# blachlylab/fade

Measured on AMD Instinct MI355X. Metric: annotate reads/sec at 1/2/4/8 MI355X; rs/am tag bit-exact vs ref, higher is better.
Workload: dtype int16; 1 GPU; C2: 10000000 x 150 bp PE reads per GPU per step in 10 distinct batches, -w 100, --min-length 5, p_softclip 0.10; slots_in_flight=2, records_left_out=none

## Files before the change

fade_amd/csrc/fadehip.hip:

```cpp
#include "fadehip_host.hpp"
#include "fadehip_kernels.hpp"
#include "sw_stats.hpp"
#include <fcntl.h>
#include <sys/stat.h>
#include <unistd.h>
#include <algorithm>
#include <cerrno>
#include <climits>
#include <cstdio>
#include <cstdlib>
#include <cstring>
#include <string>
#include <thread>
#include <vector>

using namespace fadehip;
using namespace fadehip::host;

namespace {

int reserve_run(fadehip_ctx *ctx, std::vector<void *> &trash, DevBuf &b, size_t bytes) {
    if (bytes <= b.cap && b.p) return 0;
    if (b.p) trash.push_back(b.p);
    b.p = nullptr;
// ... 219 lines not shown
    int64_t chunk_oct = 1;
    int total_oct = 0;
    uint64_t wave_stride = 0;
    int p2_waves = 1;
    size_t ckpt_bytes = 0, fwd_bytes = 0, trace_bytes = 0, cand_bytes = 0;
};

int plan_two_pass(fadehip_ctx *ctx, const Slot &s, const ClassRun &c, TwoPassPlan &p) {
    const int cls = c.cls, R = class_rows(cls), max_lr = c.max_lr, n_items = c.n_bound;
    p.n_ck = s.use_ckpt ? (max_lr + 15 + CK_COLS - 1) / CK_COLS : 0;
    p.ck_stride = (uint64_t)p.n_ck * ck_dwords(R) * 64;
    p.n_blocks1 = (max_lr + 15 + 3) / 4;
    p.ref_stride1 = std::min((((p.n_blocks1 * 4) * 2 + 15) / 16) * 16, (CH_COLS + 16) * 2);
    p.lds1 = (size_t)p.ref_stride1 * 4;
    const bool alt_rules = (ctx->sc.rules & (FADEHIP_RULE_HDIR_DIAG_F_E | FADEHIP_RULE_GAP_TIE_EXTENDS)) !=
                           (FADEHIP_RULE_HDIR_DIAG_F_E | FADEHIP_RULE_GAP_TIE_EXTENDS);
    p.mode2 = alt_rules ? 3 : 2;
    const int64_t ck_bytes = (int64_t)p.ck_stride * 4;
    p.total_oct = (n_items + 7) / 8;
    p.chunk_oct = std::max<int64_t>(1, std::min<int64_t>(p.total_oct, (c.budget / 2) / std::max<int64_t>(ck_bytes, 1)));
    p.wave_stride = (uint64_t)p.n_blocks1 * R * 64;
    p.longw = p.n_blocks1 > CH_BLOCKS;
    const int resident = resident_waves(ctx, cls, p.mode2, p.lds1, p.longw);
    const int bound_waves = (int)std::min<int64_t>(p.chunk_oct + NUM_BUCKETS, resident);
    int p2_waves = s.p2_last_octs[cls] >= 0 ? std::min(2 * s.p2_last_octs[cls] + 64, bound_waves) : std::min(1024, bound_waves);
    if (ctx->p2_waves_fixed > 0) p2_waves = std::min(ctx->p2_waves_fixed, bound_waves);
    p.p2_waves = (int)std::max<int64_t>(1, std::min<int64_t>(p2_waves, (c.budget / 2) / std::max<int64_t>((int64_t)p.wave_stride * 4, 1)));
    p.ckpt_bytes = (size_t)(p.chunk_oct * ck_bytes);
    p.fwd_bytes = (size_t)n_items * sizeof(Fwd);
    p.trace_bytes = (size_t)p.p2_waves * (size_t)p.wave_stride * 4;
    p.cand_bytes = sizeof(Cand) * (size_t)NUM_BUCKETS * (size_t)std::min<int64_t>(n_items, p.chunk_oct * 8);
    return 0;
}

int run_class_two_pass(fadehip_ctx *ctx, Slot &s, hipStream_t st, const ClassRun &c) {
    const int cls = c.cls, n_items = c.n_bound;
    TwoPassPlan p;
    int rc;
    if ((rc = plan_two_pass(ctx, s, c, p))) return rc;
    if ((rc = reserve_run(ctx, s.trash, s.ckpt, p.ckpt_bytes)) || (rc = reserve_run(ctx, s.trash, s.fwd, p.fwd_bytes)) ||
        (rc = reserve_run(ctx, s.trash, s.trace, p.trace_bytes)) || (rc = reserve_run(ctx, s.trash, s.cand, p.cand_bytes)))
        return rc;
    s.prof_counts[2] = std::max<int64_t>(s.prof_counts[2], (int64_t)p.trace_bytes);
    uint32_t *const sel_counters = s.d_sel(cls);
    const void *const score_fn = sw_kernel(cls, 1, p.longw), *const trace_fn = sw_kernel(cls, p.mode2, p.longw);
    if (!score_fn || !trace_fn) return set_err(ctx, FADEHIP_E_INVALID, "bad class %d", cls);
    bool framed = false;
    const void *const g8_fn = !p.longw && p.n_ck == 0 ? g8_kernel(ctx, cls, s.max_lq, 4 * p.n_blocks1, &framed) : nullptr;
    if (p.total_oct > p.chunk_oct) s.early = false;
    const bool early = s.early;
    for (int64_t o0 = 0; o0 < p.total_oct; o0 += p.chunk_oct) {
        const int octs = (int)std::min<int64_t>(p.chunk_oct, p.total_oct - o0);
        const int i0 = (int)(o0 * 8);
        const int n = std::min(n_items - i0, octs * 8);
        if (!s.sel_fresh[cls]) HIPCHK(ctx, hipMemsetAsync(sel_counters, 0, sizeof(uint32_t) * NUM_BUCKETS, st));
        s.sel_fresh[cls] = false;
        SwArgs a = sw_args(ctx, s, c, i0, n);
        a.ref_stride = p.ref_stride1;
        a.ckpt = (uint32_t *)s.ckpt.p;
        a.ck_stride = p.ck_stride;
        a.n_ck = p.n_ck;
        a.count_dev = c.count_dev;
        a.item_base = (uint32_t)i0;
        a.sel.enabled = 1;
        a.sel.no_ckpt = p.n_ck == 0 ? 1 : 0;
        a.sel.meta = c.meta ? c.meta + i0 : nullptr;
// ... 16 lines not shown
            HIPCHK(ctx, hipStreamWaitEvent(sst, s.ev[ef], 0));
        }
        ChunkSpans sp{c.timed};
        if ((rc = sp.mark(ctx, s, 0, sst))) return rc;
        const void *fn1 = score_fn;
        int waves1 = octs;
        size_t lds = p.lds1;
        if (ctx->score_persist && class_rows(cls) == 10 && !p.longw && s.tickets_used < (int)Slot::N_TICKETS) {
            const int res = resident_waves(ctx, cls, 1, p.lds1, p.longw);
            const int cus = std::max(ctx->cu_count, 1), mine = s.score_stream ? std::max(cus - 8 * ctx->tail_cus_per_xcd, 1) : cus;
            fn1 = (const void *)sw_pk_kernel<10, 1, false, 16, true>;
            waves1 = std::max(1, std::min(octs, (int)((int64_t)res * mine / cus)));
            a.ticket = s.d_ticket(s.tickets_used++);
        } else if (g8_fn) {
            if (ctx->debug && o0 == 0) fprintf(stderr, "[fadehip] class of %d rows: score pass on eight-lane groups (longest read of the batch: %d), column-drift frame %s\n", 16 * class_rows(cls), s.max_lq, framed ? "on" : "off");
            fn1 = g8_fn;
            waves1 = (n + 15) / 16;
            lds = 2 * p.lds1;
        }
        if ((rc = launch_sw(ctx, fn1, waves1, lds, sst, a))) return rc;
        if ((rc = sp.mark(ctx, s, 1, sst))) return rc;
        hipStream_t p2st = st;
        if (sst != st || early) {
            int ej = sp.e[1];
            if (ej < 0 && (rc = record(ctx, s, &ej, sst))) return rc;
            if (sst != st) HIPCHK(ctx, hipStreamWaitEvent(st, s.ev[ej], 0));
            if (early) {
                if (s.tail_stream) {
                    p2st = s.tail_stream;
                    HIPCHK(ctx, hipStreamWaitEvent(p2st, s.ev[ej], 0));
                }
                HIPCHK(ctx, hipMemcpyAsync(s.res.p + s.res_aln_off, s.aln.p, sizeof(fadehip_aln) * (size_t)s.out_cap, hipMemcpyDeviceToHost,
                                           s.tail_stream ? st : sst));
            }
        }
        if (s.tickets_used >= (int)Slot::N_TICKETS)
            return set_err(ctx, FADEHIP_E_UNSUPPORTED, "more than %d pass-2 launches in one run (raise trace_bytes)", (int)Slot::N_TICKETS);
        SwArgs b2 = a;
        b2.sel.enabled = 0;
        b2.n_items = 0;
        b2.cand = (const Cand *)s.cand.p;
        b2.cand_cap = (uint32_t)n;
        b2.bucket_n = sel_counters;
        b2.cand_total = &s.d_plan()->cand_total;
        b2.trace = (uint32_t *)s.trace.p;
        b2.quad_stride = p.wave_stride;
        b2.count_dev = nullptr;
        b2.ticket = s.d_ticket(s.tickets_used++);
        b2.meta = c.meta ? c.meta + i0 : nullptr;
        b2.out = c.out;
        b2.rs = c.rs;
        b2.stats = (c.rs && c.gate) ? s.d_stats() : nullptr;
        b2.floor_len = c.floor_len;
        b2.gate = c.gate;
        b2.early_out = (c.gate && c.meta && !ctx->prm.trace_all) ? 1 : 0;
        b2.rerun_total = &s.d_plan()->rerun_total;
        if ((rc = launch_sw(ctx, trace_fn, std::min(p.p2_waves, octs + NUM_BUCKETS), p.lds1, p2st, b2))) return rc;
        if ((rc = sp.mark(ctx, s, 2, p2st))) return rc;
        if (early) {
            PatchArgs pa;
            pa.cand = b2.cand;
            pa.cand_cap = b2.cand_cap;
            pa.bucket_n = sel_counters;
            pa.work = b2.work;
            pa.out = c.out;
            pa.out_cap = s.out_cap;
            pa.head = (PatchHead *)s.patch.p;
            pa.list = (PatchEntry *)((uint8_t *)s.patch.p + sizeof(PatchHead));
            pa.cap = s.patch_cap;
            const uint32_t blocks = std::max<uint32_t>(1, std::min<uint32_t>(64, (s.patch_sent * (uint32_t)(sizeof(PatchEntry) / 4) + 255) / 256));
            hipLaunchKernelGGL(patch_gather_kernel, dim3(blocks), dim3(256), 0, p2st, pa);
            HIPCHK(ctx, hipGetLastError());
            int et = -1;
            if ((rc = record(ctx, s, &et, s.tail_stream ? p2st : sst))) return rc;
            HIPCHK(ctx, hipStreamWaitEvent(st, s.ev[et], 0));
        }
    }
    return 0;
}

int run_class_single(fadehip_ctx *ctx, Slot &s, hipStream_t st, const ClassRun &c) {
    const int cls = c.cls, R = class_rows(cls), n_items = c.n_bound, max_lr = c.max_lr;
    const bool packed = ctx->use_packed;
    const int per_wave = packed ? 8 : 4;
    const int n_blocks = (max_lr + 15 + 3) / 4;
    const uint64_t quad_stride = (uint64_t)n_blocks * (packed ? R : R / 2) * 64;
    const int ref_stride = packed ? std::min((((n_blocks * 4) * 2 + 15) / 16) * 16, (CH_COLS + 16) * 2) : (((n_blocks * 4) + 15) / 16) * 16;
    const size_t lds = (size_t)ref_stride * 4;
    if (lds > 64 * 1024)
        return set_err(ctx, FADEHIP_E_UNSUPPORTED, "reference window of %d bases needs %zu B LDS per wave (max 64 KiB)", max_lr, lds);
    const int64_t quad_bytes = (int64_t)quad_stride * 4;
    int64_t max_quads = std::max<int64_t>(1, c.budget / quad_bytes);
    const int total_quads = (n_items + per_wave - 1) / per_wave;
    const int64_t chunk_quads = std::min<int64_t>(max_quads, total_quads);
    int rc = reserve_run(ctx, s.trash, s.trace, (size_t)(chunk_quads * quad_bytes));
    if (rc) return rc;
    rc = reserve_run(ctx, s.trash, s.fwd, (size_t)n_items * sizeof(Fwd));
    if (rc) return rc;
    const void *const fn = sw_kernel(cls, packed ? 0 : SW_INT32, n_blocks > CH_BLOCKS);
    if (!fn) return set_err(ctx, FADEHIP_E_INVALID, "bad class %d", cls);
    for (int64_t q0 = 0; q0 < total_quads; q0 += chunk_quads) {
        const int quads = (int)std::min<int64_t>(chunk_quads, total_quads - q0);
// ... 327 lines not shown
    if (const char *kv = getenv("FADEHIP_CKPT")) s.use_ckpt = atoi(kv) != 0;
    if (ctx->two_pass) {
        size_t need_ckpt = 0, need_fwd = 0, need_trace = 0, need_cand = 0;
        for (int c = 0; c < NUM_CLASSES; c++) {
            if (!s.bound[c]) continue;
            TwoPassPlan p;
            if ((rc = plan_two_pass(ctx, s, level2_class_run(ctx, s, c, budget), p))) return rc;
            need_ckpt = std::max(need_ckpt, p.ckpt_bytes);
            need_fwd = std::max(need_fwd, p.fwd_bytes);
            need_trace = std::max(need_trace, p.trace_bytes);
            need_cand = std::max(need_cand, p.cand_bytes);
        }
        if ((rc = reserve_run(ctx, s.trash, s.ckpt, need_ckpt)) || (rc = reserve_run(ctx, s.trash, s.fwd, need_fwd)) ||
            (rc = reserve_run(ctx, s.trash, s.trace, need_trace)) || (rc = reserve_run(ctx, s.trash, s.cand, need_cand)))
            return rc;
    }
    {
        int n_cls = 0;
        for (int c = 0; c < NUM_CLASSES; c++) n_cls += s.bound[c] ? 1 : 0;
        const char *why = nullptr;
        if (!ctx->early_copy) why = "FADEHIP_EARLY_COPY=0";
        else if (!ctx->two_pass) why = "single-pass kernels";
        else if (s.device_only) why = "results stay on the device";
        else if (n_cls != 1) why = "not exactly one class list";
        else if (s.bound[LONG_LIST]) why = "long list";
        else if (ctx->prm.trace_all) why = "trace_all";
        else if (s.last_cand * 2 > ctx->patch_cap) why = "the previous run's candidates exceed half the patch list";
        else if (s.use_ckpt) why = "snapshots";
        else if (!total_bound) why = "no alignments";
        s.early = why == nullptr;
        if (s.early) {
            s.patch_cap = (uint32_t)ctx->patch_cap;
            s.patch_sent = (uint32_t)std::min<int64_t>(s.patch_cap, 2 * s.last_cand + 64);
            const size_t bytes = sizeof(PatchHead) + sizeof(PatchEntry) * (size_t)std::max<uint32_t>(s.patch_cap, 1);
            if (((ctx->early_tail || !s.score_stream) && (rc = ensure_tail(ctx, s))) || (rc = reserve(ctx, s.patch, bytes)) ||
                (rc = reserve_pinned(ctx, s.h_patch, bytes)))
                return rc;
        }
        if (ctx->debug)
            fprintf(stderr, "[fadehip] copy order: %s (%s)\n", s.early ? "early" : "late",
                    !s.early ? why : !s.tail_stream ? "the copy on the score stream" : ctx->early_tail == 1 && !s.score_mask.empty() ? "pass 2 on the CUs the score mask leaves free" : "pass 2 on a plain stream");
    }
    if (s.zb_next_clean) s.zoff ^= Slot::ZB_STRIDE;
    else HIPCHK(ctx, hipMemsetAsync(s.zb(), 0, Slot::ZB_BYTES, st));
    s.zb_next_clean = false;
    for (int c = 0; c < NUM_CLASSES; c++) s.sel_fresh[c] = true;
    if ((rc = record(ctx, s, &s.ev_gate0))) return rc;
    GateArgs g;
    memset(&g, 0, sizeof g);
    g.n_reads = n;
    g.tid = d_arr<int32_t>(s, A_TID);
    g.pos = d_arr<int32_t>(s, A_POS);
    g.l_seq = d_arr<int32_t>(s, A_LSEQ);
    g.flag = d_arr<uint16_t>(s, A_FLAG);
    g.has_sa = d_arr<uint8_t>(s, A_SA);
    g.cigar_off = d_arr<uint32_t>(s, A_CIGOFF);
    g.cigar_ops = d_arr<uint32_t>(s, A_CIG);
    g.seq_off = d_arr<uint32_t>(s, A_SEQOFF);
    g.floor_len = floor_len;
    g.window = s.window;
    g.n_contigs = ctx->n_contigs;
    g.contig_len = (const int64_t *)ctx->contig_len.p;
    g.contig_base = (const uint64_t *)ctx->contig_base.p;
    g.max_ref_len = ctx->prm.max_ref_len;
    g.wave_lr_bound = s.wave_lr_bound;
    g.long_lr_bound = s.long_max_lr;
    g.long_lq_bound = std::max(s.long_max_lq, 1);
    g.l_seq_lo = s.l_seq_lo;
    g.l_seq_hi = s.l_seq_hi;
    g.rs = (uint8_t *)s.rs.p;
    for (int c = 0; c < NUM_LISTS; c++) {
        g.work[c] = (Work *)s.work[c].p;
        g.meta[c] = (Meta *)s.meta[c].p;
        g.list_cap[c] = s.bound[c];
    }
    g.out_cap = s.out_cap;
    g.n_cigar_ops = (uint32_t)(s.L.bytes[A_CIG] / 4);
    g.n_seq_bytes = (uint32_t)s.L.bytes[A_SEQ];
    g.stats = s.d_stats();
    g.counters = s.d_counters();
    g.counters64 = s.d_counters64();
    hipLaunchKernelGGL(gate_kernel, dim3((n + GATE_BLOCK - 1) / GATE_BLOCK), dim3(GATE_BLOCK), 0, st, g);
    HIPCHK(ctx, hipGetLastError());
    if ((rc = record(ctx, s, &s.ev_gate1))) return rc;
    uint32_t exact[NUM_LISTS];
    for (int c = 0; c < NUM_LISTS; c++) exact[c] = s.bound[c];
    if (!ctx->two_pass) {
        HIPCHK(ctx, hipMemcpyAsync(s.h_zb, s.zb(), 128, hipMemcpyDeviceToHost, st));
        HIPCHK(ctx, hipStreamSynchronize(st));
        for (int c = 0; c < NUM_LISTS; c++) exact[c] = std::min(s.h_counters()[c], s.bound[c]);
    }
    for (int c = 0; c < NUM_CLASSES; c++) {
        if (!exact[c]) continue;
        ClassRun cr = level2_class_run(ctx, s, c, budget);
        cr.n_bound = (int)exact[c];
        rc = ctx->two_pass ? run_class_two_pass(ctx, s, st, cr) : run_class_single(ctx, s, st, cr);
        if (rc) return rc;
    }
    if (exact[LONG_LIST]) {
        ClassRun cr = level2_class_run(ctx, s, LONG_LIST, budget);
        cr.n_bound = (int)exact[LONG_LIST];
        if ((rc = run_long(ctx, s, st, cr, std::max(s.long_max_lq, 1)))) return rc;
    }
    if ((rc = record(ctx, s, &s.ev_end))) return rc;
    HIPCHK(ctx, hipMemcpyAsync(s.h_zb, s.zb(), Slot::ZB_BYTES, hipMemcpyDeviceToHost, st));
    HIPCHK(ctx, hipMemsetAsync((uint8_t *)s.zblock.p + (s.zoff ^ Slot::ZB_STRIDE), 0, Slot::ZB_BYTES, st));
    s.zb_next_clean = true;
    if (s.device_only) return 0;
    HIPCHK(ctx, hipMemcpyAsync(s.res.p, s.rs.p, (size_t)n, hipMemcpyDeviceToHost, st));
    if (s.early)
        HIPCHK(ctx, hipMemcpyAsync(s.h_patch.p, s.patch.p, sizeof(PatchHead) + sizeof(PatchEntry) * (size_t)s.patch_sent, hipMemcpyDeviceToHost, st));
    else if (total_bound)
        HIPCHK(ctx, hipMemcpyAsync(s.res.p + s.res_aln_off, s.aln.p, sizeof(fadehip_aln) * (size_t)total_bound, hipMemcpyDeviceToHost, st));
    return 0;
}

int finish_run(fadehip_ctx *ctx, Slot &s, int slot) {
    if (s.state == 3) return 0;
    if (s.state != 2) return set_err(ctx, FADEHIP_E_STATE, "slot %d has not been run", slot);
    hipStream_t st = s.stream;
    const int n = s.n_reads;
    if (n == 0) {
        s.n_aln = 0;
        s.n_oversize = 0;
        memset(s.stats, 0, sizeof s.stats);
        s.stats[0] = s.n_skipped;
        s.state = 3;
        return 0;
    }
    HIPCHK(ctx, hipStreamSynchronize(st));
    for (void *q : s.trash) (void)hipFree(q);
    s.trash.clear();
    const uint32_t errbits = s.h_counters()[2 * NUM_LISTS];
    if (errbits) {
        s.state = 0;
        if (errbits & 64u) return set_err(ctx, FADEHIP_E_INVALID, "batch has a record whose cigar_off / seq_off are not non-decreasing within the arrays, or l_seq < 0");
        if (errbits & 8u) return set_err(ctx, FADEHIP_E_INVALID, "batch has a mapped soft-clipped record whose seq_packed slice is shorter than its l_seq");
        if (errbits & 16u) return set_err(ctx, FADEHIP_E_INVALID, "batch has a record whose cigar.alignedLength exceeds ref_span_bound=%lld", (long long)s.span_bound);
        if (errbits & 32u) return set_err(ctx, FADEHIP_E_INVALID, "batch has more records to re-align than its bounds said, or a read outside them (n_with_seq too small, or an l_seq outside l_seq_min / l_seq_max?)");
        return set_err(ctx, FADEHIP_E_INVALID, "batch has a mapped soft-clipped read whose tid is not a contig of the uploaded genome");
    }
    if (s.early) {
        s.early = false;
        const PatchHead head = *(const PatchHead *)s.h_patch.p;
        const PatchEntry *const list = (const PatchEntry *)(s.h_patch.p + sizeof(PatchHead));
        uint8_t *const h_aln = s.res.p + s.res_aln_off;
        if (head.overflow || head.n > s.patch_cap) {
            HIPCHK(ctx, hipMemcpyAsync(h_aln, s.aln.p, sizeof(fadehip_aln) * (size_t)s.out_cap, hipMemcpyDeviceToHost, st));
            HIPCHK(ctx, hipStreamSynchronize(st));
        } else {
            if (head.n > s.patch_sent) {
                HIPCHK(ctx, hipMemcpyAsync((void *)(list + s.patch_sent), (const uint8_t *)s.patch.p + sizeof(PatchHead) + sizeof(PatchEntry) * (size_t)s.patch_sent,
                                           sizeof(PatchEntry) * (size_t)(head.n - s.patch_sent), hipMemcpyDeviceToHost, st));
                HIPCHK(ctx, hipStreamSynchronize(st));
            }
            for (uint32_t k = 0; k < head.n; k++)
                if (list[k].out < s.out_cap) memcpy(h_aln + sizeof(fadehip_aln) * (size_t)list[k].out, &list[k].e, sizeof(fadehip_aln));
        }
        if (ctx->debug)
            fprintf(stderr, "[fadehip] slot %d: patch list of %u entries (%u sent with the run)%s\n", slot, head.n, s.patch_sent,
                    head.overflow ? ", overflow: the array was copied again" : "");
    }
    for (int c = 0; c < NUM_CLASSES; c++)
        if (s.bound[c]) {
            const uint32_t *bn = (const uint32_t *)(s.h_zb + Slot::ZB_SEL + Slot::ZB_SEL_STRIDE * (size_t)c);
            int octs = 0;
            for (int b = 0; b < NUM_BUCKETS; b++) octs += (int)((bn[b] + 7) / 8);
            s.p2_last_octs[c] = octs;
        }
    const uint32_t at = std::min(s.h_counters()[2 * NUM_LISTS + 3], s.out_cap);
    s.n_aln = (int)at;
    s.n_oversize = (int)s.h_counters()[2 * NUM_LISTS + 2];
    for (int k = 0; k < 8; k++) {
        s.stats[k] = 0;
        for (int q = 0; q < STAT_PARTS; q++) s.stats[k] += (int64_t)s.h_stats()[8 * q + k];
    }
    s.stats[0] += s.n_skipped;
    const PlanOut *po = s.h_plan();
    s.n_cand = (int64_t)po->cand_total;
    s.n_rerun = (int64_t)po->rerun_total;
    s.last_cand = s.n_cand;
    s.last_aln = (int64_t)at;
    s.prof_counts[0] = at;
    s.prof_counts[1] = (int64_t)s.h_counters64()[0 * C64_STRIDE];
    s.prof_counts[3] = (int64_t)s.h_counters64()[1 * C64_STRIDE] + (int64_t)at * 80;
    s.prof_counts[4] = ctx->two_pass ? (s.use_ckpt ? (int64_t)s.h_counters64()[2 * C64_STRIDE] : 0) : (int64_t)(s.h_counters64()[0 * C64_STRIDE] / 2);
    s.prof_counts[5] = s.n_cand;
    if (ctx->debug)
        fprintf(stderr, "[fadehip] slot %d: %d reads, %u alignments, %lld candidates traced, %lld re-run, trace need %lld B\n", slot, n, at,
                (long long)s.n_cand, (long long)s.n_rerun, (long long)s.prof_counts[2]);
// ... 821 lines not shown
```

fade_amd/csrc/fadehip_kernels.hpp:

```cpp
#pragma once
#include <type_traits>
#include <hip/hip_runtime.h>
#include <stdint.h>
#include "../../include/fadehip.h"
#include "fadehip_types.hpp"

namespace fadehip {

__host__ __device__ constexpr uint64_t make_class_lut() {
    uint64_t v = 0;
    for (int k = 0; k < 16; k++) {
        uint64_t c = 5;
        if (k == 1) c = 0;
        if (k == 2) c = 1;
        if (k == 4) c = 2;
        if (k == 8) c = 3;
        if (k == 15) c = 4;
        v |= c << (4 * k);
    }
    return v;
}
__host__ __device__ constexpr uint64_t make_comp_lut() {
    const int t[16] = {0, 8, 4, 12, 2, 10, 6, 14, 1, 9, 5, 13, 3, 11, 7, 15};
    uint64_t v = 0;
// ... 124 lines not shown
static_assert(CK_SHIFT >= 5 && CK_SHIFT <= 9, "snapshots fall on key-window ends");
__host__ __device__ constexpr int ck_dwords(int R) { return 2 * R + 4; }
constexpr int NUM_BUCKETS = 10;
__host__ __device__ constexpr int bucket_cols(int b) {
    constexpr int t[NUM_BUCKETS] = {32, 48, 64, 96, 128, 192, 256, 384, 512, 1 << 30};
    return t[b];
}

struct GateArgs {
    int32_t n_reads;
    const int32_t *tid, *pos, *l_seq;
    const uint16_t *flag;
    const uint8_t *has_sa;
    const uint32_t *cigar_off, *cigar_ops, *seq_off;
    int32_t floor_len, window;
    int32_t n_contigs;
    const int64_t *contig_len;
    const uint64_t *contig_base;
    int32_t max_ref_len;
    int32_t wave_lr_bound;
    int32_t long_lr_bound, long_lq_bound;
    int32_t l_seq_lo, l_seq_hi;
    uint32_t list_cap[NUM_LISTS];
    uint32_t out_cap;
    uint32_t n_cigar_ops, n_seq_bytes;
    uint8_t *rs;
    Work *work[NUM_LISTS];
    Meta *meta[NUM_LISTS];
    uint32_t *counters;
    unsigned long long *counters64;
    unsigned long long *stats;
};

constexpr int GATE_BLOCK = 1024;
__global__ __launch_bounds__(GATE_BLOCK) void gate_kernel(GateArgs a) {
    const int i = blockIdx.x * blockDim.x + threadIdx.x;
    unsigned long long cells = 0, seq_bytes = 0, ck_bytes = 0;
    uint32_t lr_for_max = 0, errbits = 0, st_bits = 0, oversize = 0;
    int cls = -1;
    Work w;
    Meta m;
    if (i < a.n_reads) {
        uint32_t c0 = a.cigar_off[i], c1 = a.cigar_off[i + 1];
        const uint32_t so0 = a.seq_off[i], so1 = a.seq_off[i + 1];
        const int32_t lq = a.l_seq[i];
        bool bad_rec = c0 > c1 || c1 > a.n_cigar_ops || so0 > so1 || so1 > a.n_seq_bytes || lq < 0;
        if (bad_rec) { errbits |= 64u; c1 = c0; }
        const bool out_of_bounds = !bad_rec && so1 > so0 && (lq < a.l_seq_lo || lq > a.l_seq_hi);
        if (out_of_bounds) errbits |= 32u;
        int n_soft = 0;
        uint32_t clipL = 0, clipR = 0;
        int64_t aligned = 0;
        bool first = true;
        for (uint32_t k = c0; k < c1; k++) {
            const uint32_t op = a.cigar_ops[k] & 15u, len = a.cigar_ops[k] >> 4;
            if (op == 4) n_soft++;
            if (FADEHIP_OP_CONSUMES_REF(op)) aligned += len;
            if (op == 5) continue;
            const bool is_sc = (op == 4);
            if (first && !is_sc) first = false;
            else if (first && is_sc) clipL = len;
            else if (is_sc) clipR = len;
        }
        const uint32_t flag = a.flag[i];
        uint8_t rs = 0;
        bool want = false;
        if (!((flag & 4u) || n_soft == 0) && !bad_rec) {
            if (clipL != 0 || clipR != 0) rs |= 1;
            if (a.has_sa[i]) rs |= 32;
            want = (clipL != 0 && (int64_t)clipL > a.floor_len) || (clipR != 0 && (int64_t)clipR > a.floor_len);
        }
        a.rs[i] = rs;
        st_bits = 4u | (rs & 1u) | ((rs >> 4) & 2u);
        const int32_t tid = a.tid[i];
        if (out_of_bounds) want = false;
        if (want && (tid < 0 || tid >= a.n_contigs)) {
            errbits |= 1u;
            want = false;
        }
        if (want && lq > 0 && so1 - so0 < (uint32_t)(lq + 1) / 2u) {
            errbits |= 8u;
            want = false;
        }
        if (want && lq > 0) {
            const int64_t pos = a.pos[i];
            int64_t start = pos - a.window;
            if (start < 0) start = 0;
            int64_t end = pos + aligned + a.window;
            if (end > a.contig_len[tid]) end = a.contig_len[tid];
            const int64_t lr = end - start;
            if (lr > 0) {
                cls = list_of_len(lq, lr);
                if (cls < 0) oversize = 1u;
                else if (lr > a.max_ref_len) { oversize = 1u; cls = -1; }
                else if (cls != LONG_LIST ? lr > a.wave_lr_bound : (lr > a.long_lr_bound || lq > a.long_lq_bound)) {
                    errbits |= 16u;
                    cls = -1;
                }
                else {
                    cells = (unsigned long long)lq * (unsigned long long)lr;
                    seq_bytes = (unsigned long long)((lq + 1) / 2 + (lr + 1) / 2);
                    ck_bytes = cls == LONG_LIST ? 0ull : (unsigned long long)lq * (unsigned long long)(lr >> CK_SHIFT) * 4ull;
                    lr_for_max = (uint32_t)lr;
                    w.r_base = a.contig_base[tid] + (uint64_t)start;
                    w.q_base = so0 * 2u;
                    w.lq = (uint32_t)lq;
                    w.lr = (uint32_t)lr;
                    w.idx = (uint32_t)i;
                    w.flags = 1u;
                    w.out = 0;
                    m.win_start = start;
                    m.clip_left = (int32_t)clipL;
                    m.clip_right = (int32_t)clipR;
                    m.aligned_len = (int32_t)aligned;
                    m.pad[0] = m.pad[1] = m.pad[2] = 0;
                }
            }
        }
    }
    __shared__ uint32_t s_cnt[NUM_LISTS], s_base[NUM_LISTS], s_maxlr[NUM_LISTS], s_err, s_items, s_maxlq, s_out_base;
    __shared__ unsigned long long s_cells, s_bytes, s_ck;
    __shared__ uint32_t s_key[GATE_BLOCK], s_rank[GATE_BLOCK], s_stat[3];
    if (threadIdx.x < NUM_LISTS) { s_cnt[threadIdx.x] = 0; s_maxlr[threadIdx.x] = 0; }
    if (threadIdx.x == 0) { s_err = 0; s_cells = 0; s_bytes = 0; s_ck = 0; s_items = 0; s_maxlq = 0; s_stat[0] = s_stat[1] = s_stat[2] = 0; }
    __syncthreads();
    uint32_t compact = 0;
    if (cls >= 0) {
        atomicAdd(&s_cnt[cls], 1u);
        atomicMax(&s_maxlr[cls], lr_for_max);
        if (cls == LONG_LIST) atomicMax(&s_maxlq, w.lq);
        compact = atomicAdd(&s_items, 1u);
        s_key[compact] = ((uint32_t)cls << 24) | lr_for_max;
    }
    if (__ballot(cells != 0)) {
        for (int sh = 32; sh >= 1; sh >>= 1) {
            cells += __shfl_xor(cells, sh, 64);
            seq_bytes += __shfl_xor(seq_bytes, sh, 64);
            ck_bytes += __shfl_xor(ck_bytes, sh, 64);
        }
        if ((threadIdx.x & 63) == 0) {
            atomicAdd(&s_cells, cells);
            atomicAdd(&s_bytes, seq_bytes);
            atomicAdd(&s_ck, ck_bytes);
        }
    }
    if (errbits) atomicOr(&s_err, errbits);
    if (oversize) atomicAdd(&a.counters[2 * NUM_LISTS + 2], 1u);
    {
        const unsigned long long m_read = __ballot(st_bits & 4u), m_sc = __ballot(st_bits & 1u), m_sup = __ballot(st_bits & 2u);
        if ((threadIdx.x & 63) == 0) {
            atomicAdd(&s_stat[0], (uint32_t)__popcll(m_read));
            if (m_sc) atomicAdd(&s_stat[1], (uint32_t)__popcll(m_sc));
            if (m_sup) atomicAdd(&s_stat[2], (uint32_t)__popcll(m_sup));
        }
    }
    __syncthreads();
    if (threadIdx.x < NUM_LISTS && s_cnt[threadIdx.x]) {
        s_base[threadIdx.x] = atomicAdd(&a.counters[threadIdx.x], s_cnt[threadIdx.x]);
        atomicMax(&a.counters[NUM_LISTS + threadIdx.x], s_maxlr[threadIdx.x]);
    }
    if (threadIdx.x == 0) {
        if (s_items) s_out_base = atomicAdd(&a.counters[2 * NUM_LISTS + 3], s_items);
        if (s_cells) {
            atomicAdd(&a.counters64[0 * C64_STRIDE], s_cells);
            atomicAdd(&a.counters64[1 * C64_STRIDE], s_bytes);
            atomicAdd(&a.counters64[2 * C64_STRIDE], s_ck);
        }
        if (s_err) atomicOr(&a.counters[2 * NUM_LISTS], s_err);
        if (s_maxlq) atomicMax(&a.counters[2 * NUM_LISTS + 1], s_maxlq);
    }
    if (threadIdx.x >= 64 && threadIdx.x < 67 && a.stats && s_stat[threadIdx.x - 64])
        atomicAdd(&a.stats[8 * (blockIdx.x % STAT_PARTS) + threadIdx.x - 64], (unsigned long long)s_stat[threadIdx.x - 64]);
    if (threadIdx.x < s_items) {
        const uint32_t me = s_key[threadIdx.x];
        const uint32_t n = s_items;
        uint32_t r = 0;
        for (uint32_t k = 0; k < n; k++) {
            const uint32_t o = s_key[k];
            r += ((o ^ me) >> 24) == 0 && (o > me || (o == me && k < threadIdx.x));
        }
        s_rank[threadIdx.x] = r;
    }
    __syncthreads();
    if (cls >= 0) {
        const uint32_t slot = s_base[cls] + s_rank[compact];
        w.out = s_out_base + compact;
        if (slot < a.list_cap[cls] && w.out < a.out_cap) {
            a.work[cls][slot] = w;
            a.meta[cls][slot] = m;
        } else atomicOr(&a.counters[2 * NUM_LISTS], 32u);
    }
}

struct SelArgs {
    const Meta *meta;
    int32_t floor_len;
    int32_t trace_all;
    int32_t span_slack;
    Cand *cand;
    uint32_t cap;
    uint32_t *bucket_n;
    fadehip_aln *out;
    uint8_t *rs;
    unsigned long long *stats;
    int32_t gate;
    int32_t match;
    int32_t mismatch;
    int32_t enabled;
    int32_t no_ckpt;
};

struct SwArgs {
    const Work *work;
    int32_t n_items;
    const uint8_t *q_nib;
    const uint8_t *r_nib;
    uint32_t *trace;
    uint64_t quad_stride;
    int32_t ref_stride;
    Fwd *fwd;
    ScoreTab sc;
    const Cand *cand;
// ... 1538 lines not shown
    if (item >= n_items) return 0u;
    if (a.packed == 3)
        return traceback_path(a, item, 0, a.trace + (uint64_t)item * a.quad_stride, 0, 0, item);
    const uint64_t trace_off = (uint64_t)(a.packed ? (item >> 3) : (item >> 2)) * a.quad_stride;
    return traceback_path(a, item, 0, a.trace + trace_off, a.packed ? ((item >> 1) & 3) : (item & 3), item & 1, item);
}

__global__ void traceback_kernel(TbArgs a) {
    const uint32_t r = traceback_one(a, (int)(blockIdx.x * blockDim.x + threadIdx.x));
    if (a.stats) add_artifact_stats(a.stats, r, blockIdx.x);
}

struct PatchHead {
    uint32_t n;
    uint32_t overflow;
    uint32_t pad[2];
};
struct PatchEntry {
    uint32_t out;
    uint32_t pad;
    fadehip_aln e;
};
static_assert(sizeof(fadehip_aln) % 4 == 0 && sizeof(PatchEntry) == 8 + sizeof(fadehip_aln), "the gather copies dwords");
struct PatchArgs {
    const Cand *cand;
    uint32_t cand_cap;
    const uint32_t *bucket_n;
    const Work *work;
    const fadehip_aln *out;
    uint32_t out_cap;
    PatchHead *head;
    PatchEntry *list;
    uint32_t cap;
};

__global__ __launch_bounds__(256) void patch_gather_kernel(PatchArgs a) {
    constexpr uint32_t ENTRY_DW = sizeof(PatchEntry) / 4;
    uint32_t first[NUM_BUCKETS + 1];
    first[0] = 0;
#pragma unroll
    for (int b = 0; b < NUM_BUCKETS; b++) first[b + 1] = first[b] + min(a.bucket_n[b], a.cand_cap);
    const uint32_t total = first[NUM_BUCKETS], live = min(total, a.cap);
    if (blockIdx.x == 0 && threadIdx.x == 0) {
        a.head->n = total;
        a.head->overflow = total > a.cap ? 1u : 0u;
        a.head->pad[0] = a.head->pad[1] = 0;
    }
    uint32_t *const dst = (uint32_t *)a.list;
    for (uint64_t at = (uint64_t)blockIdx.x * blockDim.x + threadIdx.x; at < (uint64_t)live * ENTRY_DW; at += (uint64_t)gridDim.x * blockDim.x) {
        const uint32_t p = (uint32_t)(at / ENTRY_DW), d = (uint32_t)(at % ENTRY_DW);
        int b = 0;
#pragma unroll
        for (int k = 1; k < NUM_BUCKETS; k++) b += p >= first[k] ? 1 : 0;
        const Cand c = a.cand[(uint64_t)b * a.cand_cap + (p - first[b])];
        const uint32_t o = a.work[c.src].out;
        uint32_t v;
        if (o >= a.out_cap) v = d == 0 ? 0xffffffffu : 0u;
        else v = d == 0 ? o : d == 1 ? 0u : ((const uint32_t *)(a.out + o))[d - 2];
        dst[at] = v;
    }
}

__global__ void set_counts_kernel(uint32_t *dst, uint32_t v) { *dst = v; }

}
```

Baseline: 1.290 billion reads/s.

## Fold rs tags and zero-block copy into early patch path; quad-vectorize gate kernel

In the early-copy path, the rs tag array is now copied to the host together with the early alignment copy. Reads whose rs byte changes during pass 2 get that byte carried in the patch entry's pad field, and the host applies it. The zero-block readback and the clearing of the next zero block move into the patch gather kernel, so the tail issues one patch memcpy instead of separate zb, memset and rs transfers. Separately, the gate kernel now handles four reads per thread with vectorized loads and a packed rs store, and uses shuffle-reduced stat counters instead of ballots. This adds complexity and relies on the early rs copy being patched correctly for bit-exact tags.

Result: faster. 1.312 billion reads/s, median of 6 (+1.7%).

```diff
diff --git a/fade_amd/csrc/fadehip.hip b/fade_amd/csrc/fadehip.hip
--- a/fade_amd/csrc/fadehip.hip
+++ b/fade_amd/csrc/fadehip.hip
@@ -275,6 +275,9 @@
     p.cand_bytes = sizeof(Cand) * (size_t)NUM_BUCKETS * (size_t)std::min<int64_t>(n_items, p.chunk_oct * 8);
     return 0;
 }
+
+constexpr size_t PATCH_ZB_OFF = sizeof(PatchHead), PATCH_LIST_OFF = PATCH_ZB_OFF + Slot::ZB_STRIDE;
+static_assert(PATCH_LIST_OFF % 16 == 0 && Slot::ZB_BYTES % 4 == 0, "the gather copies dwords; entries stay 16-byte aligned");
 
 int run_class_two_pass(fadehip_ctx *ctx, Slot &s, hipStream_t st, const ClassRun &c) {
     const int cls = c.cls, n_items = c.n_bound;
@@ -357,6 +360,7 @@
                 }
                 HIPCHK(ctx, hipMemcpyAsync(s.res.p + s.res_aln_off, s.aln.p, sizeof(fadehip_aln) * (size_t)s.out_cap, hipMemcpyDeviceToHost,
                                            s.tail_stream ? st : sst));
+                HIPCHK(ctx, hipMemcpyAsync(s.res.p, c.rs, (size_t)s.n_reads, hipMemcpyDeviceToHost, s.tail_stream ? st : sst));
             }
         }
         if (s.tickets_used >= (int)Slot::N_TICKETS)
@@ -391,8 +395,14 @@
             pa.out = c.out;
             pa.out_cap = s.out_cap;
             pa.head = (PatchHead *)s.patch.p;
-            pa.list = (PatchEntry *)((uint8_t *)s.patch.p + sizeof(PatchHead));
+            pa.list = (PatchEntry *)((uint8_t *)s.patch.p + PATCH_LIST_OFF);
             pa.cap = s.patch_cap;
+            pa.rs = c.rs;
+            pa.zb = (const uint32_t *)s.zb();
+            pa.zb_out = (uint32_t *)((uint8_t *)s.patch.p + PATCH_ZB_OFF);
+            pa.zb_next = (uint32_t *)((uint8_t *)s.zblock.p + (s.zoff ^ Slot::ZB_STRIDE));
+            pa.zb_dwords = (uint32_t)(Slot::ZB_BYTES / 4);
+            s.zb_next_clean = true;
             const uint32_t blocks = std::max<uint32_t>(1, std::min<uint32_t>(64, (s.patch_sent * (uint32_t)(sizeof(PatchEntry) / 4) + 255) / 256));
             hipLaunchKernelGGL(patch_gather_kernel, dim3(blocks), dim3(256), 0, p2st, pa);
             HIPCHK(ctx, hipGetLastError());
@@ -786,7 +796,7 @@
         if (s.early) {
             s.patch_cap = (uint32_t)ctx->patch_cap;
             s.patch_sent = (uint32_t)std::min<int64_t>(s.patch_cap, 2 * s.last_cand + 64);
-            const size_t bytes = sizeof(PatchHead) + sizeof(PatchEntry) * (size_t)std::max<uint32_t>(s.patch_cap, 1);
+            const size_t bytes = PATCH_LIST_OFF + sizeof(PatchEntry) * (size_t)std::max<uint32_t>(s.patch_cap, 1);
             if (((ctx->early_tail || !s.score_stream) && (rc = ensure_tail(ctx, s))) || (rc = reserve(ctx, s.patch, bytes)) ||
                 (rc = reserve_pinned(ctx, s.h_patch, bytes)))
                 return rc;
@@ -834,7 +844,7 @@
     g.stats = s.d_stats();
     g.counters = s.d_counters();
     g.counters64 = s.d_counters64();
-    hipLaunchKernelGGL(gate_kernel, dim3((n + GATE_BLOCK - 1) / GATE_BLOCK), dim3(GATE_BLOCK), 0, st, g);
+    hipLaunchKernelGGL(gate_kernel, dim3((n + GATE_TILE - 1) / GATE_TILE), dim3(GATE_BLOCK), 0, st, g);
     HIPCHK(ctx, hipGetLastError());
     if ((rc = record(ctx, s, &s.ev_gate1))) return rc;
     uint32_t exact[NUM_LISTS];
@@ -857,14 +867,16 @@
         if ((rc = run_long(ctx, s, st, cr, std::max(s.long_max_lq, 1)))) return rc;
     }
     if ((rc = record(ctx, s, &s.ev_end))) return rc;
+    if (s.early) {
+        HIPCHK(ctx, hipMemcpyAsync(s.h_patch.p, s.patch.p, PATCH_LIST_OFF + sizeof(PatchEntry) * (size_t)s.patch_sent, hipMemcpyDeviceToHost, st));
+        return 0;
+    }
     HIPCHK(ctx, hipMemcpyAsync(s.h_zb, s.zb(), Slot::ZB_BYTES, hipMemcpyDeviceToHost, st));
     HIPCHK(ctx, hipMemsetAsync((uint8_t *)s.zblock.p + (s.zoff ^ Slot::ZB_STRIDE), 0, Slot::ZB_BYTES, st));
     s.zb_next_clean = true;
     if (s.device_only) return 0;
     HIPCHK(ctx, hipMemcpyAsync(s.res.p, s.rs.p, (size_t)n, hipMemcpyDeviceToHost, st));
-    if (s.early)
-        HIPCHK(ctx, hipMemcpyAsync(s.h_patch.p, s.patch.p, sizeof(PatchHead) + sizeof(PatchEntry) * (size_t)s.patch_sent, hipMemcpyDeviceToHost, st));
-    else if (total_bound)
+    if (total_bound)
         HIPCHK(ctx, hipMemcpyAsync(s.res.p + s.res_aln_off, s.aln.p, sizeof(fadehip_aln) * (size_t)total_bound, hipMemcpyDeviceToHost, st));
     return 0;
 }
@@ -885,6 +897,7 @@
     HIPCHK(ctx, hipStreamSynchronize(st));
     for (void *q : s.trash) (void)hipFree(q);
     s.trash.clear();
+    if (s.early) memcpy(s.h_zb, s.h_patch.p + PATCH_ZB_OFF, Slot::ZB_BYTES);
     const uint32_t errbits = s.h_counters()[2 * NUM_LISTS];
     if (errbits) {
         s.state = 0;
@@ -897,19 +910,23 @@
     if (s.early) {
         s.early = false;
         const PatchHead head = *(const PatchHead *)s.h_patch.p;
-        const PatchEntry *const list = (const PatchEntry *)(s.h_patch.p + sizeof(PatchHead));
+        const PatchEntry *const list = (const PatchEntry *)(s.h_patch.p + PATCH_LIST_OFF);
         uint8_t *const h_aln = s.res.p + s.res_aln_off;
         if (head.overflow || head.n > s.patch_cap) {
             HIPCHK(ctx, hipMemcpyAsync(h_aln, s.aln.p, sizeof(fadehip_aln) * (size_t)s.out_cap, hipMemcpyDeviceToHost, st));
+            HIPCHK(ctx, hipMemcpyAsync(s.res.p, s.rs.p, (size_t)n, hipMemcpyDeviceToHost, st));
             HIPCHK(ctx, hipStreamSynchronize(st));
         } else {
             if (head.n > s.patch_sent) {
-                HIPCHK(ctx, hipMemcpyAsync((void *)(list + s.patch_sent), (const uint8_t *)s.patch.p + sizeof(PatchHead) + sizeof(PatchEntry) * (size_t)s.patch_sent,
+                HIPCHK(ctx, hipMemcpyAsync((void *)(list + s.patch_sent), (const uint8_t *)s.patch.p + PATCH_LIST_OFF + sizeof(PatchEntry) * (size_t)s.patch_sent,
                                            sizeof(PatchEntry) * (size_t)(head.n - s.patch_sent), hipMemcpyDeviceToHost, st));
                 HIPCHK(ctx, hipStreamSynchronize(st));
             }
             for (uint32_t k = 0; k < head.n; k++)
-                if (list[k].out < s.out_cap) memcpy(h_aln + sizeof(fadehip_aln) * (size_t)list[k].out, &list[k].e, sizeof(fadehip_aln));
+                if (list[k].out < s.out_cap) {
+                    memcpy(h_aln + sizeof(fadehip_aln) * (size_t)list[k].out, &list[k].e, sizeof(fadehip_aln));
+                    if ((uint32_t)list[k].e.read_idx < (uint32_t)n) s.res.p[list[k].e.read_idx] = (uint8_t)list[k].pad;
+                }
         }
         if (ctx->debug)
             fprintf(stderr, "[fadehip] slot %d: patch list of %u entries (%u sent with the run)%s\n", slot, head.n, s.patch_sent,
diff --git a/fade_amd/csrc/fadehip_kernels.hpp b/fade_amd/csrc/fadehip_kernels.hpp
--- a/fade_amd/csrc/fadehip_kernels.hpp
+++ b/fade_amd/csrc/fadehip_kernels.hpp
@@ -180,105 +180,171 @@
     unsigned long long *stats;
 };
 
-constexpr int GATE_BLOCK = 1024;
+constexpr int GATE_TILE = 1024, GATE_QUAD = 4, GATE_BLOCK = GATE_TILE / GATE_QUAD;
+
+template <typename T>
+__device__ __forceinline__ void gate_load_quad(const T *__restrict__ p, int r0, int nv, bool whole, T (&o)[GATE_QUAD]) {
+    typedef T V __attribute__((ext_vector_type(GATE_QUAD)));
+    if (whole && ((uintptr_t)p & (sizeof(V) - 1)) == 0) {
+        const V v = *reinterpret_cast<const V *>(p + r0);
+#pragma unroll
+        for (int k = 0; k < GATE_QUAD; k++) o[k] = v[k];
+    } else {
+#pragma unroll
+        for (int k = 0; k < GATE_QUAD; k++) o[k] = k < nv ? p[r0 + k] : T(0);
+    }
+}
+__device__ __forceinline__ void gate_load_offsets(const uint32_t *__restrict__ p, int r0, int nv, bool whole, uint32_t (&o)[GATE_QUAD + 1]) {
+    typedef uint32_t V __attribute__((ext_vector_type(GATE_QUAD)));
+    if (whole && ((uintptr_t)p & (sizeof(V) - 1)) == 0) {
+        const V v = *reinterpret_cast<const V *>(p + r0);
+#pragma unroll
+        for (int k = 0; k < GATE_QUAD; k++) o[k] = v[k];
+        o[GATE_QUAD] = p[r0 + GATE_QUAD];
+    } else {
+#pragma unroll
+        for (int k = 0; k <= GATE_QUAD; k++) o[k] = (nv > 0 && k <= nv) ? p[r0 + k] : 0u;
+    }
+}
+
 __global__ __launch_bounds__(GATE_BLOCK) void gate_kernel(GateArgs a) {
-    const int i = blockIdx.x * blockDim.x + threadIdx.x;
+    const int tile0 = blockIdx.x * GATE_TILE, r0 = tile0 + GATE_QUAD * (int)threadIdx.x;
+    const bool whole = tile0 + GATE_TILE <= a.n_reads;
+    const int nv = whole ? GATE_QUAD : max(0, min(GATE_QUAD, a.n_reads - r0));
     unsigned long long cells = 0, seq_bytes = 0, ck_bytes = 0;
-    uint32_t lr_for_max = 0, errbits = 0, st_bits = 0, oversize = 0;
-    int cls = -1;
-    Work w;
-    Meta m;
-    if (i < a.n_reads) {
-        uint32_t c0 = a.cigar_off[i], c1 = a.cigar_off[i + 1];
-        const uint32_t so0 = a.seq_off[i], so1 = a.seq_off[i + 1];
-        const int32_t lq = a.l_seq[i];
-        bool bad_rec = c0 > c1 || c1 > a.n_cigar_ops || so0 > so1 || so1 > a.n_seq_bytes || lq < 0;
-        if (bad_rec) { errbits |= 64u; c1 = c0; }
-        const bool out_of_bounds = !bad_rec && so1 > so0 && (lq < a.l_seq_lo || lq > a.l_seq_hi);
-        if (out_of_bounds) errbits |= 32u;
-        int n_soft = 0;
-        uint32_t clipL = 0, clipR = 0;
-        int64_t aligned = 0;
-        bool first = true;
-        for (uint32_t k = c0; k < c1; k++) {
-            const uint32_t op = a.cigar_ops[k] & 15u, len = a.cigar_ops[k] >> 4;
-            if (op == 4) n_soft++;
-            if (FADEHIP_OP_CONSUMES_REF(op)) aligned += len;
+    uint32_t errbits = 0, st_cnt = 0;
+    int32_t tid[GATE_QUAD], pos[GATE_QUAD], lq[GATE_QUAD];
+    uint16_t flag[GATE_QUAD];
+    uint8_t has_sa[GATE_QUAD];
+    uint32_t co[GATE_QUAD + 1], so[GATE_QUAD + 1];
+    gate_load_offsets(a.cigar_off, r0, nv, whole, co);
+    gate_load_offsets(a.seq_off, r0, nv, whole, so);
+    gate_load_quad(a.l_seq, r0, nv, whole, lq);
+    gate_load_quad(a.flag, r0, nv, whole, flag);
+    gate_load_quad(a.has_sa, r0, nv, whole, has_sa);
+    gate_load_quad(a.tid, r0, nv, whole, tid);
+    gate_load_quad(a.pos, r0, nv, whole, pos);
+    uint32_t n_ops[GATE_QUAD], max_ops = 0;
+    bool bad_rec[GATE_QUAD], out_of_bounds[GATE_QUAD];
+#pragma unroll
+    for (int k = 0; k < GATE_QUAD; k++) {
+        const bool v = k < nv;
+        bad_rec[k] = v && (co[k] > co[k + 1] || co[k + 1] > a.n_cigar_ops || so[k] > so[k + 1] || so[k + 1] > a.n_seq_bytes || lq[k] < 0);
+        if (bad_rec[k]) errbits |= 64u;
+        n_ops[k] = (v && !bad_rec[k]) ? co[k + 1] - co[k] : 0u;
+        max_ops = max(max_ops, n_ops[k]);
+        out_of_bounds[k] = v && !bad_rec[k] && so[k + 1] > so[k] && (lq[k] < a.l_seq_lo || lq[k] > a.l_seq_hi);
+        if (out_of_bounds[k]) errbits |= 32u;
+    }
+    int n_soft[GATE_QUAD];
+    uint32_t clipL[GATE_QUAD], clipR[GATE_QUAD];
+    int64_t aligned[GATE_QUAD];
+    bool first[GATE_QUAD];
+#pragma unroll
+    for (int k = 0; k < GATE_QUAD; k++) { n_soft[k] = 0; clipL[k] = clipR[k] = 0; aligned[k] = 0; first[k] = true; }
+    for (uint32_t j = 0; j < max_ops; j++) {
+        uint32_t c[GATE_QUAD];
+#pragma unroll
+        for (int k = 0; k < GATE_QUAD; k++) c[k] = j < n_ops[k] ? a.cigar_ops[co[k] + j] : 0u;
+#pragma unroll
+        for (int k = 0; k < GATE_QUAD; k++) {
+            if (j >= n_ops[k]) continue;
+            const uint32_t op = c[k] & 15u, len = c[k] >> 4;
+            if (op == 4) n_soft[k]++;
+            if (FADEHIP_OP_CONSUMES_REF(op)) aligned[k] += len;
             if (op == 5) continue;
             const bool is_sc = (op == 4);
-            if (first && !is_sc) first = false;
-            else if (first && is_sc) clipL = len;
-            else if (is_sc) clipR = len;
-        }
-        const uint32_t flag = a.flag[i];
-        uint8_t rs = 0;
-        bool want = false;
-        if (!((flag & 4u) || n_soft == 0) && !bad_rec) {
-            if (clipL != 0 || clipR != 0) rs |= 1;
-            if (a.has_sa[i]) rs |= 32;
-            want = (clipL != 0 && (int64_t)clipL > a.floor_len) || (clipR != 0 && (int64_t)clipR > a.floor_len);
-        }
-        a.rs[i] = rs;
-        st_bits = 4u | (rs & 1u) | ((rs >> 4) & 2u);
-        const int32_t tid = a.tid[i];
-        if (out_of_bounds) want = false;
-        if (want && (tid < 0 || tid >= a.n_contigs)) {
+            if (first[k] && !is_sc) first[k] = false;
+            else if (first[k] && is_sc) clipL[k] = len;
+            else if (is_sc) clipR[k] = len;
+        }
+    }
+    uint32_t rs4 = 0;
+    bool want[GATE_QUAD];
+#pragma unroll
+    for (int k = 0; k < GATE_QUAD; k++) {
+        uint32_t rs = 0;
+        want[k] = false;
+        if (k < nv && !((flag[k] & 4u) || n_soft[k] == 0) && !bad_rec[k]) {
+            if (clipL[k] != 0 || clipR[k] != 0) rs |= 1;
+            if (has_sa[k]) rs |= 32;
+            want[k] = (clipL[k] != 0 && (int64_t)clipL[k] > a.floor_len) || (clipR[k] != 0 && (int64_t)clipR[k] > a.floor_len);
+        }
+        rs4 |= rs << (8 * k);
+        if (k < nv) st_cnt += 1u | ((rs & 1u) << 10) | ((rs >> 5) << 20);
+        if (out_of_bounds[k]) want[k] = false;
+        if (want[k] && (tid[k] < 0 || tid[k] >= a.n_contigs)) {
             errbits |= 1u;
-            want = false;
-        }
-        if (want && lq > 0 && so1 - so0 < (uint32_t)(lq + 1) / 2u) {
+            want[k] = false;
+        }
+        if (want[k] && lq[k] > 0 && so[k + 1] - so[k] < (uint32_t)(lq[k] + 1) / 2u) {
             errbits |= 8u;
-            want = false;
-        }
-        if (want && lq > 0) {
-            const int64_t pos = a.pos[i];
-            int64_t start = pos - a.window;
-            if (start < 0) start = 0;
-            int64_t end = pos + aligned + a.window;
-            if (end > a.contig_len[tid]) end = a.contig_len[tid];
-            const int64_t lr = end - start;
-            if (lr > 0) {
-                cls = list_of_len(lq, lr);
-                if (cls < 0) oversize = 1u;
-                else if (lr > a.max_ref_len) { oversize = 1u; cls = -1; }
-                else if (cls != LONG_LIST ? lr > a.wave_lr_bound : (lr > a.long_lr_bound || lq > a.long_lq_bound)) {
-                    errbits |= 16u;
-                    cls = -1;
-                }
-                else {
-                    cells = (unsigned long long)lq * (unsigned long long)lr;
-                    seq_bytes = (unsigned long long)((lq + 1) / 2 + (lr + 1) / 2);
-                    ck_bytes = cls == LONG_LIST ? 0ull : (unsigned long long)lq * (unsigned long long)(lr >> CK_SHIFT) * 4ull;
-                    lr_for_max = (uint32_t)lr;
-                    w.r_base = a.contig_base[tid] + (uint64_t)start;
-                    w.q_base = so0 * 2u;
-                    w.lq = (uint32_t)lq;
-                    w.lr = (uint32_t)lr;
-                    w.idx = (uint32_t)i;
-                    w.flags = 1u;
-                    w.out = 0;
-                    m.win_start = start;
-                    m.clip_left = (int32_t)clipL;
-                    m.clip_right = (int32_t)clipR;
-                    m.aligned_len = (int32_t)aligned;
-                    m.pad[0] = m.pad[1] = m.pad[2] = 0;
-                }
-            }
-        }
+            want[k] = false;
+        }
+        want[k] = want[k] && lq[k] > 0;
+    }
+    if (whole && ((uintptr_t)a.rs & 3) == 0) *reinterpret_cast<uint32_t *>(a.rs + r0) = rs4;
+    else {
+#pragma unroll
+        for (int k = 0; k < GATE_QUAD; k++)
+            if (k < nv) a.rs[r0 + k] = (uint8_t)(rs4 >> (8 * k));
+    }
+    int64_t c_len[GATE_QUAD];
+    uint64_t c_base[GATE_QUAD];
+#pragma unroll
+    for (int k = 0; k < GATE_QUAD; k++) {
+        c_len[k] = want[k] ? a.contig_len[tid[k]] : 0;
+        c_base[k] = want[k] ? a.contig_base[tid[k]] : 0;
+    }
+    int cls[GATE_QUAD];
+    uint32_t lr_of[GATE_QUAD];
+    int64_t start_of[GATE_QUAD];
+#pragma unroll
+    for (int k = 0; k < GATE_QUAD; k++) {
+        cls[k] = -1;
+        lr_of[k] = 0;
+        start_of[k] = 0;
+        if (!want[k]) continue;
+        int64_t start = (int64_t)pos[k] - a.window;
+        if (start < 0) start = 0;
+        int64_t end = (int64_t)pos[k] + aligned[k] + a.window;
+        if (end > c_len[k]) end = c_len[k];
+        const int64_t lr = end - start;
+        if (lr <= 0) continue;
+        int c = list_of_len(lq[k], lr);
+        bool oversize = false;
+        if (c < 0) oversize = true;
+        else if (lr > a.max_ref_len) { oversize = true; c = -1; }
+        else if (c != LONG_LIST ? lr > a.wave_lr_bound : (lr > a.long_lr_bound || lq[k] > a.long_lq_bound)) {
+            errbits |= 16u;
+            c = -1;
+        } else {
+            cells += (unsigned long long)lq[k] * (unsigned long long)lr;
+            seq_bytes += (unsigned long long)((lq[k] + 1) / 2 + (lr + 1) / 2);
+            ck_bytes += c == LONG_LIST ? 0ull : (unsigned long long)lq[k] * (unsigned long long)(lr >> CK_SHIFT) * 4ull;
+            lr_of[k] = (uint32_t)lr;
+            start_of[k] = start;
+        }
+        if (oversize) atomicAdd(&a.counters[2 * NUM_LISTS + 2], 1u);
+        cls[k] = c;
     }
     __shared__ uint32_t s_cnt[NUM_LISTS], s_base[NUM_LISTS], s_maxlr[NUM_LISTS], s_err, s_items, s_maxlq, s_out_base;
     __shared__ unsigned long long s_cells, s_bytes, s_ck;
-    __shared__ uint32_t s_key[GATE_BLOCK], s_rank[GATE_BLOCK], s_stat[3];
+    __shared__ uint32_t s_key[GATE_TILE], s_rank[GATE_TILE], s_stat[3];
     if (threadIdx.x < NUM_LISTS) { s_cnt[threadIdx.x] = 0; s_maxlr[threadIdx.x] = 0; }
     if (threadIdx.x == 0) { s_err = 0; s_cells = 0; s_bytes = 0; s_ck = 0; s_items = 0; s_maxlq = 0; s_stat[0] = s_stat[1] = s_stat[2] = 0; }
     __syncthreads();
-    uint32_t compact = 0;
-    if (cls >= 0) {
-        atomicAdd(&s_cnt[cls], 1u);
-        atomicMax(&s_maxlr[cls], lr_for_max);
-        if (cls == LONG_LIST) atomicMax(&s_maxlq, w.lq);
-        compact = atomicAdd(&s_items, 1u);
-        s_key[compact] = ((uint32_t)cls << 24) | lr_for_max;
+    uint32_t compact[GATE_QUAD];
+#pragma unroll
+    for (int k = 0; k < GATE_QUAD; k++) {
+        compact[k] = 0;
+        if (cls[k] >= 0) {
+            atomicAdd(&s_cnt[cls[k]], 1u);
+            atomicMax(&s_maxlr[cls[k]], lr_of[k]);
+            if (cls[k] == LONG_LIST) atomicMax(&s_maxlq, (uint32_t)lq[k]);
+            compact[k] = atomicAdd(&s_items, 1u);
+            s_key[compact[k]] = ((uint32_t)cls[k] << 24) | lr_of[k];
+        }
     }
     if (__ballot(cells != 0)) {
         for (int sh = 32; sh >= 1; sh >>= 1) {
@@ -293,13 +359,13 @@
         }
     }
     if (errbits) atomicOr(&s_err, errbits);
-    if (oversize) atomicAdd(&a.counters[2 * NUM_LISTS + 2], 1u);
     {
-        const unsigned long long m_read = __ballot(st_bits & 4u), m_sc = __ballot(st_bits & 1u), m_sup = __ballot(st_bits & 2u);
+        for (int sh = 32; sh >= 1; sh >>= 1) st_cnt += __shfl_xor(st_cnt, sh, 64);
         if ((threadIdx.x & 63) == 0) {
-            atomicAdd(&s_stat[0], (uint32_t)__popcll(m_read));
-            if (m_sc) atomicAdd(&s_stat[1], (uint32_t)__popcll(m_sc));
-            if (m_sup) atomicAdd(&s_stat[2], (uint32_t)__popcll(m_sup));
+            const uint32_t n_read = st_cnt & 1023u, n_sc = (st_cnt >> 10) & 1023u, n_sup = st_cnt >> 20;
+            if (n_read) atomicAdd(&s_stat[0], n_read);
+            if (n_sc) atomicAdd(&s_stat[1], n_sc);
+            if (n_sup) atomicAdd(&s_stat[2], n_sup);
         }
     }
     __syncthreads();
@@ -319,23 +385,41 @@
     }
     if (threadIdx.x >= 64 && threadIdx.x < 67 && a.stats && s_stat[threadIdx.x - 64])
         atomicAdd(&a.stats[8 * (blockIdx.x % STAT_PARTS) + threadIdx.x - 64], (unsigned long long)s_stat[threadIdx.x - 64]);
-    if (threadIdx.x < s_items) {
-        const uint32_t me = s_key[threadIdx.x];
+    {
         const uint32_t n = s_items;
-        uint32_t r = 0;
-        for (uint32_t k = 0; k < n; k++) {
-            const uint32_t o = s_key[k];
-            r += ((o ^ me) >> 24) == 0 && (o > me || (o == me && k < threadIdx.x));
-        }
-        s_rank[threadIdx.x] = r;
+        for (uint32_t t = threadIdx.x; t < n; t += GATE_BLOCK) {
+            const uint32_t me = s_key[t];
+            uint32_t r = 0;
+            for (uint32_t k = 0; k < n; k++) {
+                const uint32_t o = s_key[k];
+                r += ((o ^ me) >> 24) == 0 && (o > me || (o == me && k < t));
+            }
+            s_rank[t] = r;
+        }
     }
     __syncthreads();
-    if (cls >= 0) {
-        const uint32_t slot = s_base[cls] + s_rank[compact];
-        w.out = s_out_base + compact;
-        if (slot < a.list_cap[cls] && w.out < a.out_cap) {
-            a.work[cls][slot] = w;
-            a.meta[cls][slot] = m;
+#pragma unroll
+    for (int k = 0; k < GATE_QUAD; k++) {
+        if (cls[k] < 0) continue;
+        const uint32_t slot = s_base[cls[k]] + s_rank[compact[k]];
+        const uint32_t out = s_out_base + compact[k];
+        if (slot < a.list_cap[cls[k]] && out < a.out_cap) {
+            Work w;
+            w.r_base = c_base[k] + (uint64_t)start_of[k];
+            w.q_base = so[k] * 2u;
+            w.lq = (uint32_t)lq[k];
+            w.lr = lr_of[k];
+            w.idx = (uint32_t)(r0 + k);
+            w.flags = 1u;
+            w.out = out;
+            Meta m;
+            m.win_start = start_of[k];
+            m.clip_left = (int32_t)clipL[k];
+            m.clip_right = (int32_t)clipR[k];
+            m.aligned_len = (int32_t)aligned[k];
+            m.pad[0] = m.pad[1] = m.pad[2] = 0;
+            a.work[cls[k]][slot] = w;
+            a.meta[cls[k]][slot] = m;
         } else atomicOr(&a.counters[2 * NUM_LISTS], 32u);
     }
 }
@@ -1940,6 +2024,11 @@
     PatchHead *head;
     PatchEntry *list;
     uint32_t cap;
+    const uint8_t *rs;
+    const uint32_t *zb;
+    uint32_t *zb_out;
+    uint32_t *zb_next;
+    uint32_t zb_dwords;
 };
 
 __global__ __launch_bounds__(256) void patch_gather_kernel(PatchArgs a) {
@@ -1954,6 +2043,11 @@
         a.head->overflow = total > a.cap ? 1u : 0u;
         a.head->pad[0] = a.head->pad[1] = 0;
     }
+    if (blockIdx.x == 0)
+        for (uint32_t d = threadIdx.x; d < a.zb_dwords; d += blockDim.x) {
+            a.zb_out[d] = a.zb[d];
+            a.zb_next[d] = 0;
+        }
     uint32_t *const dst = (uint32_t *)a.list;
     for (uint64_t at = (uint64_t)blockIdx.x * blockDim.x + threadIdx.x; at < (uint64_t)live * ENTRY_DW; at += (uint64_t)gridDim.x * blockDim.x) {
         const uint32_t p = (uint32_t)(at / ENTRY_DW), d = (uint32_t)(at % ENTRY_DW);
@@ -1964,7 +2058,7 @@
         const uint32_t o = a.work[c.src].out;
         uint32_t v;
         if (o >= a.out_cap) v = d == 0 ? 0xffffffffu : 0u;
-        else v = d == 0 ? o : d == 1 ? 0u : ((const uint32_t *)(a.out + o))[d - 2];
+        else v = d == 0 ? o : d == 1 ? (uint32_t)a.rs[a.work[c.src].idx] : ((const uint32_t *)(a.out + o))[d - 2];
         dst[at] = v;
     }
 }
```
